# Happy-ZZX/PL-VIWO

Hardware: AMD Instinct MI355X
Metric: frames/sec (track+EKF update), 752x480 mono, 250 pts+80 lines; ATE vs CPU ref (higher is better)
Workload: dtype f64

## Files before the change

include/plviwo.h:

```cpp
#ifndef PLVIWO_H
#define PLVIWO_H

#include <stddef.h>
#include <stdint.h>

#ifdef __cplusplus
extern "C" {
#endif

#if defined(__GNUC__)
#pragma GCC visibility push(default)
#endif

#define PLV_ABI_VERSION 1

enum {
  PLV_OK = 0,
  PLV_E_BADARG = -1,
  PLV_E_DEVICE = -2,
  PLV_E_NOT_PSD = -3,
  PLV_E_NOMEM = -4,
  PLV_E_CAPACITY = -5,
  PLV_E_NO_DEVICE = -6,
  PLV_E_NUMERIC = -7
// ... 224 lines not shown
  const double *line_FinG;
  const int *D;
  const double *anchor_pt;
  const uint8_t *has_pt;
  const double *res_R;
  const double *res_p;
  const double *res_Q;
  const int *res_clone;
} plv_line_tracks;

int plv_triangulate_lines(plv_ctx *ctx, const plv_state_view *st, const plv_line_tracks *lt, double *line_FinG,
                          uint8_t *ok);

int plv_line_segments(plv_ctx *ctx, const plv_state_view *st, const plv_line_tracks *lt, double *end_points ,
                      double *extent , int *n_views , uint8_t *ok );

int plv_line_jacobian_columns(const plv_state_view *st, const plv_line_tracks *lt, int *col_to_state, int cap, int *k_out);

int plv_build_line_jacobians(plv_ctx *ctx, const plv_state_view *st, const plv_line_tracks *lt, int k,
                             const int *col_to_state, int ld, int *rows, double *Hf, double *Hx, double *res);
int plv_build_line_jacobians_resident(plv_ctx *ctx, const plv_state_view *st, const plv_line_tracks *lt, int k,
                                      const int *col_to_state, int ld);

int plv_detect_lines(plv_ctx *ctx, int which, float *lines, int cap, int *n_out);
int plv_line_prefetch_mode(plv_ctx *ctx, int on);
int plv_line_worker_config(int spin_us, int fit_threads, int *spin_us_out, int *fit_threads_out);
int plv_line_tracker_feed_async(plv_ctx *ctx, double timestamp, const double *vps);
int plv_line_tracker_feed_wait(plv_ctx *ctx);
int plv_line_detect_launch(plv_ctx *ctx, int which);
int plv_line_detect_finish(plv_ctx *ctx, int which);
int plv_line_walk_mode(plv_ctx *ctx, int on_device);
int plv_line_walk_info(plv_ctx *ctx, int *mode, int *n_components, int *longest_component, int *n_chains, int *fell_back);
int plv_line_chains(plv_ctx *ctx, int cap_chains, int cap_pts, int *chain_ptr, int *pts_xy, int *n_chains);

int plv_assign_points_to_lines(const float *lines, int n_lines, const float *pts, const uint64_t *ids, int n_pts, int *kept,
                               int *rel_ptr, uint64_t *rel_id, double *rel_dist, int *pos_ptr, float *pos_xy, int *n_kept);
int plv_line_match(const float *lines_new, int n_new, const int *rel_ptr_new, const uint64_t *rel_id_new, const float *lines_last,
                   int n_last, const int *rel_ptr_last, const uint64_t *rel_id_last, int *match_of_new);
int plv_line_classification(const float *line, const double *vps);
int plv_vanishing_points(const double *R_ItoC, const double *K8, double *vps);

int plv_line_tracker_feed(plv_ctx *ctx, double timestamp, const double *vps);
int plv_line_tracker_feed_points(plv_ctx *ctx, double timestamp, const double *vps, int n, const float *pts, const uint64_t *ids);
int plv_line_tracker_last(plv_ctx *ctx, float *lines, uint64_t *ids, int cap, int *n);
int plv_line_db_size(plv_ctx *ctx);
int plv_line_db_ids(plv_ctx *ctx, uint64_t *ids, int cap, int *n);
int plv_line_db_export_tracks(plv_ctx *ctx, const uint64_t *ids, int n_ids, int *obs_ptr, double *obs_time, float *seg_uv,
                              float *seg_uvn, int obs_cap, int *D, int *pts_ptr, int *pt_ids, int pts_cap);
int plv_line_db_remove(plv_ctx *ctx, const uint64_t *ids, int n_ids);

int plv_db_append_measurements(plv_ctx *ctx, uint64_t id, int n, const double *t, const float *uv, const float *uvn);

typedef struct plv_update_options {
  int max_msckf;
  int max_obs;
  double chi2_mult;
  plv_tri_options tri;
  double t_prev_frame;
  double state_time;
  int window_full;
  int max_slam;
  int n_slam;
  const uint64_t *slam_ids;
  int init_min_meas;
  const plv_cpi_table *cpi;
} plv_update_options;
// ... 278 lines not shown
```

pl-viwo_amd/__init__.py:

```python
import ctypes as C
import os

import numpy as np

_HERE = os.path.dirname(os.path.abspath(__file__))
LIB_PATH = os.path.join(_HERE, "lib", "libplviwo_hip.so")

PLV_OK = 0
PLV_E_BADARG = -1
PLV_E_DEVICE = -2
PLV_E_NOT_PSD = -3
PLV_E_NOMEM = -4
PLV_E_CAPACITY = -5
PLV_E_NO_DEVICE = -6
PLV_E_NUMERIC = -7

PLV_CAM_RADTAN = 0
PLV_CAM_EQUIDISTANT = 1
ENCODINGS = {"mono8": 0, "bayer_rggb8": 1, "bayer_bggr8": 2, "bayer_gbrg8": 3, "bayer_grbg8": 4, "bgr8": 5, "rgb8": 6, "bgra8": 7,
             "rgba8": 8}
_ENC_BPP = (1, 1, 1, 1, 1, 3, 3, 4, 4)


class PlvConfig(C.Structure):
# ... 188 lines not shown
        "plv_debug_knobs": (C.c_uint, [C.c_longlong]),
        "plv_chain_count": (C.c_ulonglong, []),
        "plv_decision_trace": (C.c_int, [C.c_void_p, C.c_int]),
        "plv_last_point_decisions": (C.c_int, [C.c_void_p, C.POINTER(C.c_uint64), C.POINTER(C.c_double), C.c_int, C.POINTER(C.c_int)]),
        "plv_last_line_decisions": (C.c_int, [C.c_void_p, C.POINTER(C.c_uint64), C.POINTER(C.c_double), C.c_int, C.POINTER(C.c_int)]),
        "plv_route_counts": (None, [C.POINTER(C.c_ulonglong)]),
        "plv_speculation_counts": (None, [C.POINTER(C.c_ulonglong)]),
        "plv_memory_bytes": (None, [C.POINTER(C.c_ulonglong)]),
        "plv_memory_policy": (C.c_int, [C.c_int, C.c_int, C.c_int]),
        "plv_alloc_count": (C.c_ulonglong, []),
        "plv_phase_counters": (None, [C.POINTER(C.c_ulonglong)]),
        "plv_camera_update_lines": (C.c_int, [vp, C.POINTER(PlvStateView), C.POINTER(PlvUpdateOptions), dp,
                                              C.POINTER(PlvUpdateResult), u64p, u8p, dp, C.c_int]),
        "plv_slam_update": (C.c_int, [vp, C.c_int, C.c_int, C.c_int, dp, dp, ip, C.c_double, u8p, dp]),
        "plv_slam_initialize": (C.c_int, [vp, C.c_int, C.c_int, C.c_int, dp, dp, dp, ip, C.c_double, u8p, dp, dp]),
        "plv_cov_marginalize": (C.c_int, [vp, C.c_int, C.c_int]),
        "plv_landmark_from_xyz": (C.c_int, [C.c_int, dp, dp]),
        "plv_landmark_xyz": (C.c_int, [C.c_int, dp, dp]),
        "plv_camera_update_slam": (C.c_int, [vp, C.POINTER(PlvStateView), C.POINTER(PlvUpdateOptions), C.c_int, vp, C.c_int, vp,
                                             C.POINTER(PlvTracks), C.POINTER(PlvSlamResult), u64p, u8p, dp]),
        "plv_camera_init_slam": (C.c_int, [vp, C.POINTER(PlvStateView), C.POINTER(PlvUpdateOptions), C.c_int, vp, ip, C.c_int, vp,
                                           C.POINTER(PlvTracks), C.POINTER(PlvSlamResult), u64p, u8p, dp]),
        "plv_detect_lines": (C.c_int, [vp, C.c_int, fp, C.c_int, ip]),
        "plv_line_detect_launch": (C.c_int, [vp, C.c_int]),
        "plv_line_detect_finish": (C.c_int, [vp, C.c_int]),
        "plv_counters": (None, [C.POINTER(C.c_ulonglong)]),
        "plv_jpl_left_update": (None, [C.c_int, dp, dp, dp]),
        "plv_state_boxplus": (C.c_int, [C.c_int, C.POINTER(PlvStateVar), dp, C.c_int]),
        "plv_camera_try_update": (C.c_int, [vp, C.POINTER(PlvStateView), C.POINTER(PlvTryUpdate)]),
        "plv_camera_frame": (C.c_int, [vp, C.POINTER(PlvStateView), C.POINTER(PlvCameraFrameIo)]),
        "plv_line_walk_mode": (C.c_int, [vp, C.c_int]),
        "plv_line_walk_info": (C.c_int, [vp, ip, ip, ip, ip, ip]),
        "plv_line_chains": (C.c_int, [vp, C.c_int, C.c_int, ip, ip, ip]),
        "plv_line_prefetch_mode": (C.c_int, [vp, C.c_int]),
        "plv_line_tracker_feed_async": (C.c_int, [vp, C.c_double, dp]),
        "plv_line_tracker_feed_wait": (C.c_int, [vp]),
        "plv_assign_points_to_lines": (C.c_int, [fp, C.c_int, fp, u64p, C.c_int, ip, ip, u64p, dp, ip, fp, ip]),
        "plv_line_match": (C.c_int, [fp, C.c_int, ip, u64p, fp, C.c_int, ip, u64p, ip]),
        "plv_line_classification": (C.c_int, [fp, dp]),
        "plv_vanishing_points": (C.c_int, [dp, dp, dp]),
        "plv_line_tracker_feed": (C.c_int, [vp, C.c_double, dp]),
        "plv_line_tracker_feed_points": (C.c_int, [vp, C.c_double, dp, C.c_int, fp, u64p]),
        "plv_line_tracker_last": (C.c_int, [vp, fp, u64p, C.c_int, ip]),
        "plv_line_tracker_last_points": (C.c_int, [vp, ip, u64p, C.c_int, C.c_int, ip]),
        "plv_draw_primitives": (C.c_int, [vp, u8p, C.c_int, C.c_int, C.c_int, C.POINTER(PlvDrawPrim), C.c_int, u8p, C.c_int, u8p, C.c_int]),
        "plv_track_image_options_default": (None, [C.POINTER(PlvTrackImageOptions)]),
        "plv_track_image": (C.c_int, [vp, C.POINTER(PlvTrackImageOptions), u8p, C.c_int]),
        "plv_track_image_primitives": (C.c_int, [vp, C.POINTER(PlvTrackImageOptions), C.POINTER(PlvDrawPrim), C.c_int, ip]),
        "plv_line_db_size": (C.c_int, [vp]),
        "plv_line_db_ids": (C.c_int, [vp, u64p, C.c_int, ip]),
        "plv_line_db_export_tracks": (C.c_int, [vp, u64p, C.c_int, ip, dp, fp, fp, C.c_int, ip, ip, ip, C.c_int]),
        "plv_line_db_remove": (C.c_int, [vp, u64p, C.c_int]),
        "plv_triangulate_lines": (C.c_int, [vp, C.POINTER(PlvStateView), C.POINTER(PlvLineTracks), dp, u8p]),
        "plv_line_segments": (C.c_int, [vp, C.POINTER(PlvStateView), C.POINTER(PlvLineTracks), dp, dp, ip, u8p]),
        "plv_line_map_mode": (C.c_int, [vp, C.c_int]),
        "plv_camera_used_lines": (C.c_int, [vp, C.POINTER(PlvStateView), C.c_int, ip, u64p, u8p, dp, dp, u8p]),
        "plv_line_jacobian_columns": (C.c_int, [C.POINTER(PlvStateView), C.POINTER(PlvLineTracks), ip, C.c_int, ip]),
        "plv_build_line_jacobians": (C.c_int, [vp, C.POINTER(PlvStateView), C.POINTER(PlvLineTracks), C.c_int, ip, C.c_int, ip,
                                               dp, dp, dp]),
        "plv_build_line_jacobians_resident": (C.c_int, [vp, C.POINTER(PlvStateView), C.POINTER(PlvLineTracks), C.c_int, ip,
                                                        C.c_int]),
    }
    for name, (res, args) in sig.items():
        fn = getattr(lib, name)
        fn.restype = res
        fn.argtypes = args
# ... 1331 lines not shown
            self._chk(self.lib.plv_last_point_decisions(self.h, ids.ctypes.data_as(C.POINTER(C.c_uint64)), vals.ctypes.data_as(C.POINTER(C.c_double)),
                                                        n.value, C.byref(n)))
        return ids, vals

    def last_line_decisions(self):
        n = C.c_int(0)
        self._chk(self.lib.plv_last_line_decisions(self.h, None, None, 0, C.byref(n)))
        ids, vals = np.zeros(n.value, dtype=np.uint64), np.zeros((n.value, 3))
        if n.value:
            self._chk(self.lib.plv_last_line_decisions(self.h, ids.ctypes.data_as(C.POINTER(C.c_uint64)), vals.ctypes.data_as(C.POINTER(C.c_double)),
                                                       n.value, C.byref(n)))
        return ids, vals

    def line_prefetch_mode(self, on):
        self._chk(self.lib.plv_line_prefetch_mode(self.h, 1 if on else 0))

    def line_walk_mode(self, on_device):
        self._chk(self.lib.plv_line_walk_mode(self.h, int(on_device)))

    def line_walk_info(self):
        v = [C.c_int() for _ in range(5)]
        self._chk(self.lib.plv_line_walk_info(self.h, *[C.byref(x) for x in v]))
        return dict(zip(("mode", "n_components", "longest_component", "n_chains", "fell_back"), (x.value for x in v)))

    def line_chains(self):
        n = C.c_int()
        self._chk(self.lib.plv_line_chains(self.h, 0, 0, None, None, C.byref(n)))
        ptr = np.zeros(n.value + 1, dtype=np.int32)
        self._chk(self.lib.plv_line_chains(self.h, n.value, 0, _ip(ptr), None, C.byref(n)))
        pts = np.zeros((max(int(ptr[-1]), 1), 2), dtype=np.int32)
        self._chk(self.lib.plv_line_chains(self.h, n.value, int(ptr[-1]), _ip(ptr), _ip(pts), C.byref(n)))
        return [pts[ptr[c]:ptr[c + 1]].copy() for c in range(n.value)]

    def assign_points_to_lines(self, lines, pts, ids):
        lines = np.ascontiguousarray(lines, dtype=np.float32).reshape(-1, 4)
        pts = np.ascontiguousarray(pts, dtype=np.float32).reshape(-1, 2)
        ids = np.ascontiguousarray(ids, dtype=np.uint64)
        nl, npt = len(lines), len(pts)
        kept = np.zeros(max(nl, 1), dtype=np.int32)
        rel_ptr, pos_ptr = np.zeros(nl + 1, dtype=np.int32), np.zeros(nl + 1, dtype=np.int32)
        rel_id, rel_d = np.zeros(nl * npt + 1, dtype=np.uint64), np.zeros(nl * npt + 1)
        pos = np.zeros((nl * npt + 1, 2), dtype=np.float32)
        nk = C.c_int()
        self._chk(self.lib.plv_assign_points_to_lines(_fp(lines), nl, _fp(pts), _u64p(ids), npt, _ip(kept), _ip(rel_ptr), _u64p(rel_id),
                                                      _dp(rel_d), _ip(pos_ptr), _fp(pos), C.byref(nk)))
        nk = nk.value
        return dict(kept=kept[:nk].copy(), rel_ptr=rel_ptr[:nk + 1].copy(), rel_id=rel_id[:rel_ptr[nk]].copy(),
                    rel_dist=rel_d[:rel_ptr[nk]].copy(), pos_ptr=pos_ptr[:nk + 1].copy(), pos=pos[:pos_ptr[nk]].copy())

    def line_match(self, lines_new, rel_ptr_new, rel_id_new, lines_last, rel_ptr_last, rel_id_last):
        ln = np.ascontiguousarray(lines_new, dtype=np.float32).reshape(-1, 4)
        ll = np.ascontiguousarray(lines_last, dtype=np.float32).reshape(-1, 4)
        rpn, rpl = _i32(rel_ptr_new), _i32(rel_ptr_last)
        rin = np.ascontiguousarray(rel_id_new, dtype=np.uint64)
        ril = np.ascontiguousarray(rel_id_last, dtype=np.uint64)
        out = np.zeros(max(1, len(ln)), dtype=np.int32)
        self._chk(self.lib.plv_line_match(_fp(ln), len(ln), _ip(rpn), _u64p(rin), _fp(ll), len(ll), _ip(rpl), _u64p(ril), _ip(out)))
        return out[:len(ln)].copy()

    def line_classification(self, line, vps):
        line = np.ascontiguousarray(line, dtype=np.float32)
        vps = np.ascontiguousarray(vps, dtype=np.float64)
        return self.lib.plv_line_classification(_fp(line), _dp(vps))

    def vanishing_points(self, R_ItoC, K8):
        R = np.ascontiguousarray(R_ItoC, dtype=np.float64)
# ... 246 lines not shown
```

pl-viwo_amd/csrc/line_api.hip:

```cpp
#include <algorithm>
#include <chrono>
#include <cmath>
#include <cstring>
#include <atomic>
#include <condition_variable>
#include <functional>
#include <memory>
#include <map>
#include <mutex>
#include <thread>
#include <unordered_map>
#include <vector>

#include "line_host.hpp"
#include "cam_models.hpp"
#include "line_kernels.hpp"
#include "update_state.hpp"
#include "plv_internal.hpp"
#include "camera_tracks.hpp"
#include "update_tail.hpp"

using namespace plv;
using namespace plv::linehost;

// ... 35 lines not shown
  std::vector<int> ptr, D, valid_n, cols, pt_ptr, pt_ids;
  std::vector<double> anchor, ot;
  std::vector<float> uv, uvn;
  std::vector<uint8_t> has, flags;
  CpiPoses cpi;
  std::vector<double> lg_two_step;
  std::vector<uint8_t> ok_two_step;
  double us_pool = 0;
  plv_line_tracks view() const {
    plv_line_tracks all{};
    all.n_lines = Lp, all.obs_ptr = ptr.data(), all.obs_time = ot.data(), all.seg_uv = uv.data(), all.seg_uvn = uvn.data();
    all.D = D.data(), all.anchor_pt = anchor.data(), all.has_pt = has.data();
    if (cpi.on && !cpi.R.empty()) all.res_R = cpi.R.data(), all.res_p = cpi.p.data();
    return all;
  }
};

struct LineTracker {
  LinePool pool_prep;
  LinesJob ujob;
  std::vector<float> lines_last;
  std::vector<uint64_t> ids_last;
  std::vector<int> rel_ptr_last{0};
  std::vector<uint64_t> rel_id_last;
  uint64_t currid = 1;
  bool walk_on_device = false;
  int walk_mode = 0;
  struct WalkInfo {
    int mode = 0, n_components = 0, longest_component = 0, n_chains = 0, fell_back = 0;
  } winfo;
  bool chains_valid = false;
  std::vector<FldChain> last_chains;
  int last_pts_extent = 0;
  DevBuf comps, recs, recs_sorted;
  bool prefetch = false;
  std::unordered_map<uint64_t, LineTrack> db;
  DevBuf half, map, work, pts, chains, counts, segs, seg_count, uv_in, uv_out;
  DevBuf lab, lab_cnt, lab_roots;
  hipStream_t ccl_stream = nullptr;
  hipEvent_t canny_done = nullptr, labels_ready = nullptr;
  PinBuf pin;
  hipEvent_t edges_ready = nullptr;
  std::vector<uint64_t> dec_ids;
  std::vector<double> dec_vals;
  struct LineMapRecord {
    std::vector<uint64_t> ids;
    std::vector<uint8_t> accepted;
    std::vector<double> lines, res_R, res_p;
    std::vector<int> sel, ptr;
    std::vector<double> ot;
    std::vector<float> uv, uvn;
  } map_rec;
  const uint8_t *early_raw = nullptr;
  const unsigned *early_hist = nullptr;
  int early_w = 0, early_h = 0;
  int pending_which = -1, pending_fed = -1;
  bool defer_finish = false;
  std::function<void()> deferred;
  std::atomic<int> defer_state{0};
  struct TriState {
    bool valid = false;
    plv_state_view view;
    std::vector<double> clone_time, clone_R, clone_p;
    std::vector<int> clone_id;
  } tri_state;
  std::vector<float> cached;
// ... 196 lines not shown
  TRY(T->work.reserve(npix));
  TRY(T->pts.reserve(npix * sizeof(int2)));
  TRY(T->chains.reserve(kChainCap * sizeof(FldChain)));
  TRY(T->counts.reserve(12 * sizeof(int)));
  const size_t slot_cap = npix / (size_t)fp.length_threshold + kChainCap;
  TRY(T->segs.reserve(slot_cap * sizeof(float4)));
  TRY(T->seg_count.reserve(kChainCap * sizeof(int)));
  FldBuffers b{T->half.as<uint8_t>(), T->map.as<uint8_t>(), T->work.as<uint8_t>(), T->pts.as<int2>(), T->chains.as<FldChain>(),
               kChainCap,             T->counts.as<int>(),  T->segs.as<float4>(), T->seg_count.as<int>()};
  const size_t bytes = 16 + kChainCap * (sizeof(FldChain) + sizeof(int));
  const size_t lab_off = bytes + ((2 * npix + 63) & ~(size_t)63) + npix * sizeof(int2);
  const size_t nblk = (npix + 255) / 256, sorted_off = (lab_off + npix + 63) & ~(size_t)63, bins_off = sorted_off + nblk * 256;
  const size_t pin_end = bins_off + nblk * (size_t)(plv::line_label_parts() + 1) * sizeof(unsigned short);
  const size_t info_off = (std::max(bytes + slot_cap * sizeof(float4), pin_end + 64) + 63) & ~(size_t)63;
  TRY(T->pin.reserve(info_off + 64));
  char *hp = T->pin.as<char>();
  const bool maps_to_host = !T->walk_on_device && fp.canny_low == fp.canny_high;
  if (maps_to_host) {
    b.map = (uint8_t *)(hp + bytes);
    b.half = b.map + npix;
  }
  const bool with_labels = launch_only && maps_to_host;
  if (with_labels) {
    TRY(T->lab.reserve(npix * sizeof(int)));
    TRY(T->lab_cnt.reserve(npix * sizeof(int)));
    TRY(T->lab_roots.reserve(plv::line_label_roots_bytes()));
    b.lab_work = T->lab.as<int>();
    b.lab_cnt = T->lab_cnt.as<int>();
    b.lab_roots = T->lab_roots.as<int>();
    b.lab_out = (uint8_t *)(hp + lab_off);
    b.blk_sorted = (uint8_t *)(hp + sorted_off);
    b.blk_bins = (unsigned short *)(hp + bins_off);
  }
  const bool comp_walk = T->walk_mode == 2 && fp.canny_low == fp.canny_high && plv::line_walk_lds_bytes(w, h) <= plv::kLineWalkLdsMax;
  if (comp_walk) {
    (void)join_job(T);
    const size_t rec_cap = npix / (size_t)(std::max(1, fp.length_threshold) + 1) + 1;
    TRY(T->lab.reserve(npix * sizeof(int)));
    TRY(T->lab_cnt.reserve(npix * sizeof(int)));
    TRY(T->lab_roots.reserve(plv::line_label_roots_bytes()));
    TRY(T->comps.reserve((size_t)plv::line_walk_components_cap() * sizeof(FldComp)));
    TRY(T->recs.reserve(rec_cap * sizeof(FldRec)));
    TRY(T->recs_sorted.reserve(rec_cap * sizeof(FldRec)));
    b.lab_work = T->lab.as<int>();
    b.lab_cnt = T->lab_cnt.as<int>();
    b.lab_roots = T->lab_roots.as<int>();
    b.comps = T->comps.as<FldComp>();
    b.recs = T->recs.as<FldRec>();
    b.recs_sorted = T->recs_sorted.as<FldRec>();
    b.walk_info = T->counts.as<int>() + 4;
  }
  if (!prelaunched) TRY(launch_line_edges(ctx, d_img, W, H, fp, b, ctx->stream, early ? T->early_hist : nullptr));
  if (with_labels && !T->ccl_stream) {
    PLV_HIP_CHECK(hipStreamCreateWithFlags(&T->ccl_stream, hipStreamNonBlocking));
    PLV_HIP_CHECK(hipEventCreateWithFlags(&T->canny_done, hipEventDisableTiming));
    PLV_HIP_CHECK(hipEventCreateWithFlags(&T->labels_ready, hipEventDisableTiming));
  }
  if (with_labels) PLV_HIP_CHECK(hipEventRecord(T->canny_done, ctx->stream));
  if (launch_only && !T->edges_ready) PLV_HIP_CHECK(hipEventCreateWithFlags(&T->edges_ready, hipEventDisableTiming));
  if (launch_only && maps_to_host) PLV_HIP_CHECK(hipEventRecord(T->edges_ready, ctx->stream));
  if (early && ctx->after_edges) TRY(ctx->after_edges(ctx->after_edges_arg));
  if (with_labels) {
    PLV_HIP_CHECK(hipStreamWaitEvent(T->ccl_stream, T->canny_done, 0));
    TRY(launch_line_labels(ctx, w, h, b, T->ccl_stream, fp.length_threshold));
    PLV_HIP_CHECK(hipEventRecord(T->labels_ready, T->ccl_stream));
  }
  const float thr2 = ctx->cfg.line_min_length_px * ctx->cfg.line_min_length_px;
  auto emit = [&](const float4 &sg) {
    const float x1 = sg.x * 2, y1 = sg.y * 2, x2 = sg.z * 2, y2 = sg.w * 2;
    const float l2 = (x2 - x1) * (x2 - x1) + (y2 - y1) * (y2 - y1);
    if (!(l2 > thr2)) return;
    lines.insert(lines.end(), {x1, y1, x2, y2});
  };
  lines.clear();
  if (!T->walk_on_device) {
    const bool timing = plv::knob(plv::PLV_KNOB_LINE_TIMING);
    if (prelaunched) {
      const bool had = join_job(T);
      if (had && T->job.rc == PLV_OK) {
        lines.swap(T->job.lines);
        return PLV_OK;
      }
      if (had && T->job.rc != PLV_OK) return T->job.rc;
    } else {
      (void)join_job(T);
    }
    plv::linehost::quiesce_helpers(T->host.fit);
    Job &J = T->job;
    J.device = ctx->device, J.w = w, J.h = h, J.length_threshold = fp.length_threshold, J.distance_threshold = fp.distance_threshold;
    J.thr2 = thr2;
    uint8_t *hmap = (uint8_t *)(hp + bytes);
    J.hmap = hmap, J.hhalf = hmap + npix;
    J.hpts = (int2 *)(hp + bytes + ((2 * npix + 63) & ~(size_t)63));
    J.hc = (FldChain *)(hp + 16);
    J.hlab = with_labels ? b.lab_out : nullptr;
    J.parts = with_labels ? plv::line_label_parts() : 0;
    J.hsorted = with_labels ? b.blk_sorted : nullptr, J.hbins = with_labels ? b.blk_bins : nullptr;
    if (!maps_to_host) {
      PLV_HIP_CHECK(plv::memcpy_async(hmap, T->map.p, npix, hipMemcpyDeviceToHost, ctx->stream));
      PLV_HIP_CHECK(plv::memcpy_async(hmap + npix, T->half.p, npix, hipMemcpyDeviceToHost, ctx->stream));
    }
    if (launch_only) {
      if (!maps_to_host) PLV_HIP_CHECK(hipEventRecord(T->edges_ready, ctx->stream));
      T->pending_which = which;
      T->pending_fed = plv_front_fed_count(ctx) + (early ? 1 : 0);
      if (!T->worker.joinable()) T->worker = std::thread(line_worker, T);
      {
        std::lock_guard<std::mutex> lk(T->jm);
        T->job_state = 1;
        T->job_posted = std::chrono::steady_clock::now();
      }
      T->jcv.notify_all();
      prewake_helpers(&T->host);
      return PLV_OK;
    }
    PLV_HIP_CHECK(plv::stream_sync(ctx->stream));
    TRY(host_extract(&T->host, J, timing));
    lines.swap(J.lines);
    ctx->prof.collect();
    return PLV_OK;
  }
  int *hinfo = (int *)(hp + info_off);
  if (comp_walk) {
    TRY(launch_line_walk_components(ctx, w, h, fp, b));
    TRY(launch_line_walk(ctx, w, h, fp, b, b.walk_info + 2));
    TRY(launch_line_fit(ctx, w, h, fp, b, b.walk_info + 2));
    PLV_HIP_CHECK(plv::memcpy_async(hinfo, b.walk_info, 8 * sizeof(int), hipMemcpyDeviceToHost, ctx->stream));
  } else {
    TRY(launch_line_walk(ctx, w, h, fp, b));
// ... 87 lines not shown
  if (n_components) *n_components = T->winfo.n_components;
  if (longest_component) *longest_component = T->winfo.longest_component;
  if (n_chains) *n_chains = T->winfo.n_chains;
  if (fell_back) *fell_back = T->winfo.fell_back;
  return PLV_OK;
}

int plv_line_chains(plv_ctx *ctx, int cap_chains, int cap_pts, int *chain_ptr, int *pts_xy, int *n_chains) {
  if (!ctx || cap_chains < 0 || cap_pts < 0) return PLV_E_BADARG;
  (void)hipSetDevice(ctx->device);
  LineTracker *T = ltr(ctx);
  std::lock_guard<std::mutex> lk(T->mtx);
  if (!T->chains_valid) {
    set_last_error("plv_line_chains: the last detection did not run on the device (plv_line_walk_mode 1 or 2)");
    return PLV_E_BADARG;
  }
  const int n = (int)T->last_chains.size();
  size_t total = 0;
  for (const FldChain &c : T->last_chains) total += (size_t)c.len;
  if (n_chains) *n_chains = n;
  if (!chain_ptr) return PLV_OK;
  if (n > cap_chains || (pts_xy && total > (size_t)cap_pts)) return PLV_E_CAPACITY;
  chain_ptr[0] = 0;
  for (int c = 0; c < n; ++c) chain_ptr[c + 1] = chain_ptr[c] + T->last_chains[c].len;
  if (!pts_xy || total == 0) return PLV_OK;
  std::vector<int2> hp((size_t)T->last_pts_extent);
  PLV_HIP_CHECK(plv::memcpy_async(hp.data(), T->pts.p, hp.size() * sizeof(int2), hipMemcpyDeviceToHost, ctx->stream));
  PLV_HIP_CHECK(plv::stream_sync(ctx->stream));
  for (int c = 0; c < n; ++c) {
    const FldChain &ch = T->last_chains[c];
    if (ch.start < 0 || (size_t)ch.start + (size_t)ch.len > hp.size()) return PLV_E_DEVICE;
    for (int q = 0; q < ch.len; ++q) pts_xy[2 * ((size_t)chain_ptr[c] + q)] = hp[(size_t)ch.start + q].x, pts_xy[2 * ((size_t)chain_ptr[c] + q) + 1] = hp[(size_t)ch.start + q].y;
  }
  return PLV_OK;
}

int plv_line_worker_config(int spin_us, int fit_threads_n, int *spin_us_out, int *fit_threads_out) {
  if (spin_us >= 0) spin_budget_us().store(spin_us);
  if (fit_threads_n >= 0) fit_threads().store(std::min(fit_threads_n, (int)plv::linehost::Fit::kThreads));
  if (spin_us_out) *spin_us_out = spin_budget_us().load();
  if (fit_threads_out) *fit_threads_out = fit_threads().load();
  return PLV_OK;
}

int plv_line_prefetch_mode(plv_ctx *ctx, int on) {
  if (!ctx) return PLV_E_BADARG;
  LineTracker *T = ltr(ctx);
  std::lock_guard<std::mutex> lk(T->mtx);
  T->prefetch = on != 0;
  return PLV_OK;
}
}
namespace plv {
int plv_line_prefetch_enabled(plv_ctx *ctx) {
  {
    std::lock_guard<std::mutex> lk(g_mtx);
    if (g_lt.find(ctx) == g_lt.end()) return 0;
  }
  LineTracker *T = ltr(ctx);
  std::lock_guard<std::mutex> lk(T->mtx);
  return T->prefetch && !T->walk_on_device ? 1 : 0;
}
}
extern "C" {

int plv_detect_lines(plv_ctx *ctx, int which, float *lines, int cap, int *n_out) {
// ... 891 lines not shown
```

pl-viwo_amd/csrc/line_kernels.hip:

```cpp
#include "line_kernels.hpp"

#include "fld_fit_core.hpp"
#include "equalize_lut.hpp"

namespace plv {

__global__ void __launch_bounds__(256) half_kernel(const uint8_t *__restrict__ src, int w, int h, uint8_t *__restrict__ dst) {
  const int w2 = w >> 1, h2 = h >> 1;
  const int x = blockIdx.x * 64 + (threadIdx.x & 63), y = blockIdx.y * 4 + (threadIdx.x >> 6);
  if (x >= w2 || y >= h2) return;
  const uint8_t *p = src + (size_t)(2 * y) * w + 2 * x;
  dst[(size_t)y * w2 + x] = (uint8_t)((p[0] + p[1] + p[w] + p[w + 1] + 2) >> 2);
}

#define CN_T 16
__device__ __forceinline__ int ccl_find(const int *L, int i) {
  for (;;) {
    const int p = __atomic_load_n(L + i, __ATOMIC_RELAXED);
    if (p == i) return i;
    i = p;
  }
}
__device__ __forceinline__ void ccl_union(int *L, int a, int b) {
  for (;;) {
// ... 85 lines not shown
    const int me = ty * CN_T + tx;
    const bool edge = inside && out == 2;
    lab[me] = edge ? me : -1;
    lcnt[me] = 0;
    __syncthreads();
    if (edge) {
      if (tx > 0 && lab[me - 1] >= 0) ccl_union(lab, me, me - 1);
      if (ty > 0) {
        if (tx > 0 && lab[me - CN_T - 1] >= 0) ccl_union(lab, me, me - CN_T - 1);
        if (lab[me - CN_T] >= 0) ccl_union(lab, me, me - CN_T);
        if (tx + 1 < CN_T && lab[me - CN_T + 1] >= 0) ccl_union(lab, me, me - CN_T + 1);
      }
    }
    __syncthreads();
    int r = -1;
    if (edge) {
      r = ccl_find(lab, me);
      atomicAdd(&lcnt[r], 1);
    }
    __syncthreads();
    if (inside) {
      lab_init[(size_t)y * w + x] = edge ? (y0 + r / CN_T) * w + x0 + (r & (CN_T - 1)) : -1;
      if (cnt_init) cnt_init[(size_t)y * w + x] = lcnt[me];
    }
  }
}

#define CCL_BIG 8
#define CCL_HASHED 16
#define CCL_ROOT_CAP 4096
#define CCL_PARTS (CCL_BIG + CCL_HASHED)
__global__ void __launch_bounds__(256) ccl_boundary_kernel(int *__restrict__ L, int w, int h, int *__restrict__ n_roots) {
  const int i = blockIdx.x * 256 + threadIdx.x;
  if (i == 0) *n_roots = 0;
  if (i >= w * h || L[i] < 0) return;
  const int y = i / w, x = i - y * w;
  const int lx = x & (CN_T - 1), ly = y & (CN_T - 1);
  if (lx == 0 && x > 0 && L[i - 1] >= 0) ccl_union(L, i, i - 1);
  if (y > 0) {
    if ((lx == 0 || ly == 0) && x > 0 && L[i - w - 1] >= 0) ccl_union(L, i, i - w - 1);
    if (ly == 0 && L[i - w] >= 0) ccl_union(L, i, i - w);
    if ((ly == 0 || lx == CN_T - 1) && x + 1 < w && L[i - w + 1] >= 0) ccl_union(L, i, i - w + 1);
  }
}
__global__ void __launch_bounds__(256) ccl_roots_kernel(int *__restrict__ L, int n, int *__restrict__ cnt, int *__restrict__ roots, int *__restrict__ n_roots) {
  const int i = blockIdx.x * 256 + threadIdx.x;
  if (i >= n || L[i] < 0) return;
  const int r = ccl_find(L, i);
  if (r != i) {
    __atomic_store_n(L + i, r, __ATOMIC_RELAXED);
    const int c = cnt[i];
    if (c > 0) {
      atomicAdd(cnt + r, c);
      cnt[i] = 0;
    }
  }
  if (r == i) {
    const int at = atomicAdd(n_roots, 1);
    if (at < CCL_ROOT_CAP) roots[at] = i;
  }
}
__global__ void __launch_bounds__(1024) ccl_assign_kernel(int *__restrict__ cnt, const int *__restrict__ roots, const int *__restrict__ n_roots, int min_px) {
  __shared__ int lsz[512], lrt[512];
  __shared__ int n_large;
  const int n = min(*n_roots, CCL_ROOT_CAP);
  const bool listed = *n_roots <= CCL_ROOT_CAP;
  if (threadIdx.x == 0) n_large = 0;
  __syncthreads();
  for (int j = threadIdx.x; j < n; j += blockDim.x) {
    const int root = roots[j], c = cnt[root];
    bool large = false;
    if (listed && c >= 64) {
      const int at = atomicAdd(&n_large, 1);
      if (at < 512) lsz[at] = c, lrt[at] = root, large = true;
    }
    if (!large) cnt[root] = c < min_px ? -255 : -(1 + CCL_BIG + (int)(((unsigned)root * 2654435761u >> 8) % (unsigned)CCL_HASHED));
  }
  __syncthreads();
  const int m = min(n_large, 512);
  for (int j = threadIdx.x; j < m; j += blockDim.x) {
    const int mine = lsz[j], root = lrt[j];
    int rank = 0;
    for (int q = 0; q < m && rank < CCL_BIG; ++q) rank += (lsz[q] > mine) || (lsz[q] == mine && lrt[q] < root);
    cnt[root] = -(rank < CCL_BIG ? 1 + rank : 1 + CCL_BIG + (int)(((unsigned)root * 2654435761u >> 8) % (unsigned)CCL_HASHED));
  }
}
__global__ void __launch_bounds__(256) ccl_flatten_kernel(const int *__restrict__ L, int n, const int *__restrict__ cnt, uint8_t *__restrict__ lab_out, int min_px,
                                                          uint8_t *__restrict__ blk_sorted, unsigned short *__restrict__ blk_bins) {
  __shared__ unsigned short wcnt[4][CCL_PARTS], start[CCL_PARTS + 1];
  const int i = blockIdx.x * 256 + threadIdx.x;
  uint8_t v = 0;
  if (i < n) {
    const int r = L[i];
    if (r >= 0) {
      const int c = cnt[r];
      v = (uint8_t)(c < 0 ? -c : (c < min_px ? 255 : 1 + CCL_BIG + (int)(((unsigned)r * 2654435761u >> 8) % (unsigned)CCL_HASHED)));
    }
    lab_out[i] = v;
  }
  if (!blk_sorted) return;
  const int part = (v >= 1 && v <= CCL_PARTS) ? v - 1 : -1, wave = threadIdx.x >> 6, lane = threadIdx.x & 63;
  int before = 0;
  for (int p = 0; p < CCL_PARTS; ++p) {
    const unsigned long long m = __ballot(part == p);
    if (part == p) before = __popcll(m & ((1ull << lane) - 1ull));
    if (lane == 0) wcnt[wave][p] = (unsigned short)__popcll(m);
  }
  __syncthreads();
  if (wave == 0) {
    int tot = lane < CCL_PARTS ? wcnt[0][lane] + wcnt[1][lane] + wcnt[2][lane] + wcnt[3][lane] : 0, inc = tot;
#pragma unroll
    for (int off = 1; off < 32; off <<= 1) {
      const int o = __shfl_up(inc, off, 64);
      if (lane >= off) inc += o;
    }
    if (lane < CCL_PARTS) start[lane + 1] = (unsigned short)inc;
    if (lane == 0) start[0] = 0;
  }
  __syncthreads();
  if (threadIdx.x <= CCL_PARTS) blk_bins[(size_t)blockIdx.x * (CCL_PARTS + 1) + threadIdx.x] = start[threadIdx.x];
  if (part >= 0) {
    int at = start[part] + before;
    for (int w = 0; w < wave; ++w) at += wcnt[w][part];
    blk_sorted[(size_t)blockIdx.x * 256 + at] = (uint8_t)threadIdx.x;
  }
}

__global__ void __launch_bounds__(1024) canny_hyst_kernel(uint8_t *__restrict__ map, int w, int h) {
  __shared__ int changed;
  do {
    __syncthreads();
    if (threadIdx.x == 0) changed = 0;
// ... 443 lines not shown
}

static inline int cdiv(int a, int b) { return (a + b - 1) / b; }

int launch_line_edges(plv_ctx *ctx, const uint8_t *d_img, int W, int H, const FldParams &fp, FldBuffers &b, hipStream_t st, const unsigned *d_hist) {
  if (!st) st = ctx->stream;
  const int w = W / 2, h = H / 2;
  int low = fp.canny_low, high = fp.canny_high;
  if (low > high) std::swap(low, high);
  {
    ProfScope ps(ctx->prof, "half_canny_kernel", st);
    hipLaunchKernelGGL(canny_kernel<true>, dim3(cdiv(w, CN_T), cdiv(h, CN_T)), dim3(CN_T * CN_T), 0, st, d_img, W, w, h, low,
                       high, b.map, b.half, d_hist, W * H, b.lab_work, b.lab_cnt);
  }
  if (low != high) {
    ProfScope ps(ctx->prof, "canny_hyst_kernel", st);
    hipLaunchKernelGGL(canny_hyst_kernel, dim3(1), dim3(1024), 0, st, b.map, w, h);
  }
  PLV_HIP_CHECK(hipGetLastError());
  return PLV_OK;
}

int launch_line_labels(plv_ctx *ctx, int w, int h, FldBuffers &b, hipStream_t st, int length_threshold) {
  const int n = w * h;
  const int min_px = length_threshold + 1;
  {
    ProfScope ps(ctx->prof, "ccl_boundary_kernel", st);
    hipLaunchKernelGGL(ccl_boundary_kernel, dim3(cdiv(n, 256)), dim3(256), 0, st, b.lab_work, w, h, b.lab_roots + CCL_ROOT_CAP);
  }
  {
    ProfScope ps(ctx->prof, "ccl_roots_kernel", st);
    hipLaunchKernelGGL(ccl_roots_kernel, dim3(cdiv(n, 256)), dim3(256), 0, st, b.lab_work, n, b.lab_cnt, b.lab_roots, b.lab_roots + CCL_ROOT_CAP);
  }
  {
    ProfScope ps(ctx->prof, "ccl_assign_kernel", st);
    hipLaunchKernelGGL(ccl_assign_kernel, dim3(1), dim3(1024), 0, st, b.lab_cnt, b.lab_roots, b.lab_roots + CCL_ROOT_CAP, min_px);
  }
  {
    ProfScope ps(ctx->prof, "ccl_flatten_kernel", st);
    hipLaunchKernelGGL(ccl_flatten_kernel, dim3(cdiv(n, 256)), dim3(256), 0, st, b.lab_work, n, b.lab_cnt, b.lab_out, min_px, b.blk_sorted, b.blk_bins);
  }
  PLV_HIP_CHECK(hipGetLastError());
  return PLV_OK;
}
int line_label_parts() { return CCL_PARTS; }
size_t line_label_roots_bytes() { return (CCL_ROOT_CAP + 4) * sizeof(int); }

int launch_line_walk(plv_ctx *ctx, int w, int h, const FldParams &fp, FldBuffers &b, const int *gate) {
  ProfScope ps(ctx->prof, "fld_walk_kernel", ctx->stream);
  const size_t need = (size_t)w * h;
  if (need <= 150 * 1024) {
    PLV_HIP_CHECK(ensure_dyn_smem((const void *)fld_walk_kernel<true>, (int)need));
    hipLaunchKernelGGL(fld_walk_kernel<true>, dim3(1), dim3(64), need, ctx->stream, b.map, w, h, fp.length_threshold, b.work, b.pts,
                       b.chains, b.chain_cap, b.counts, gate);
  } else {
    hipLaunchKernelGGL(fld_walk_kernel<false>, dim3(1), dim3(64), 0, ctx->stream, b.map, w, h, fp.length_threshold, b.work, b.pts,
                       b.chains, b.chain_cap, b.counts, gate);
  }
  PLV_HIP_CHECK(hipGetLastError());
  return PLV_OK;
}

int launch_line_fit(plv_ctx *ctx, int w, int h, const FldParams &fp, FldBuffers &b, const int *gate) {
  ProfScope ps(ctx->prof, "fld_fit_kernel", ctx->stream);
  hipLaunchKernelGGL(fld_fit_kernel, dim3(cdiv(b.chain_cap, 64)), dim3(64), 0, ctx->stream, b.half, w, h, fp.length_threshold,
                     fp.distance_threshold, b.pts, b.chains, b.counts, b.segs, b.seg_count, gate);
  PLV_HIP_CHECK(hipGetLastError());
  return PLV_OK;
}

size_t line_walk_lds_bytes(int w, int h) { return (size_t)h * (size_t)((w + 63) / 64) * sizeof(unsigned long long); }
int line_walk_components_cap() { return CCL_ROOT_CAP; }
int launch_line_walk_components(plv_ctx *ctx, int w, int h, const FldParams &fp, FldBuffers &b) {
  hipStream_t st = ctx->stream;
  const int n = w * h, min_px = fp.length_threshold + 1;
  const size_t lds = line_walk_lds_bytes(w, h);
  if (lds > kLineWalkLdsMax || !b.lab_work || !b.comps) return PLV_E_BADARG;
  {
    ProfScope ps(ctx->prof, "ccl_boundary_kernel", st);
// ... 36 lines not shown
```

pl-viwo_amd/csrc/plv_ctx.hpp:

```cpp
#pragma once
#include <hip/hip_runtime.h>
#include <sys/resource.h>

#include "gate_stage.hpp"
#include <cstdint>
#include <cstdio>
#include <execinfo.h>
#include <cstring>
#include <algorithm>
#include <atomic>
#include <chrono>
#include <cstdlib>
#include <mutex>
#include <string>
#include <unordered_map>
#include <vector>

#include "../../include/plviwo.h"

namespace plv {

void set_last_error(const char *fmt, ...);

#define PLV_HIP_CHECK(expr)                                                              \
// ... 15 lines not shown
  std::atomic<unsigned long long> speculated{0};
  std::atomic<unsigned long long> route[8] = {};
};
inline Counters &counters() {
  static Counters c;
  return c;
}
inline int spec_grid(int max_sel) { return 2 * (max_sel > 0 ? max_sel : 1); }
inline hipError_t stream_sync(hipStream_t s) {
  ++counters().syncs;
  return hipStreamSynchronize(s);
}
inline hipError_t event_sync(hipEvent_t e) {
  ++counters().syncs;
  return hipEventSynchronize(e);
}
inline hipError_t memcpy_async(void *dst, const void *src, size_t bytes, hipMemcpyKind kind, hipStream_t s) {
  ++counters().copies;
  counters().copy_bytes += bytes;
  return hipMemcpyAsync(dst, src, bytes, kind, s);
}

enum : unsigned { PLV_KNOB_PRIOR_LATE = 2u, PLV_KNOB_GATE_SEPARATE = 1024u, PLV_KNOB_NO_CHAIN = 2048u, PLV_KNOB_CHAIN_ALWAYS = 4096u,
                  PLV_KNOB_FORCE_FACTOR_FORM = 8192u,
                  PLV_KNOB_HOST_TIMING = 1u << 14,
                  PLV_KNOB_LINE_TIMING = 1u << 15,
                  PLV_KNOB_UPDATE_TIMING = 1u << 16,
                  PLV_KNOB_KERNEL_STAMPS = 1u << 17,
                  PLV_KNOB_CHAIN_EVENTS = 1u << 18,
                  PLV_KNOB_ALLOC_DEBUG = 1u << 19,
                  PLV_KNOB_HOST_FAULTS = 1u << 20,
                  PLV_KNOB_NO_SPECULATION = 1u << 24,
                  PLV_KNOB_HELPER_NAPS = 1u << 28,
                  PLV_KNOB_TSQR_TREE = 1u << 29 };
inline std::atomic<unsigned> &knobs() {
  static std::atomic<unsigned> k{getenv("PLV_DEBUG_KNOBS") ? (unsigned)strtoul(getenv("PLV_DEBUG_KNOBS"), nullptr, 0) : 0u};
  return k;
}
inline bool knob(unsigned bit) { return (knobs().load(std::memory_order_relaxed) & bit) != 0; }
inline bool alloc_debug() { return knob(PLV_KNOB_ALLOC_DEBUG); }

struct HostPhases {
  struct Rec {
    const char *label;
    double us = 0;
    long n = 0;
    float last[64] = {};
    void put(double v) {
      last[n & 63] = (float)v;
      us += v;
      ++n;
    }
    double median() const {
      float tmp[64];
      const int m = (int)(n < 64 ? n : 64);
      for (int i = 0; i < m; ++i) tmp[i] = last[i];
      std::sort(tmp, tmp + m);
      return m ? tmp[m / 2] : 0.0;
    }
  };
  bool on = knob(PLV_KNOB_HOST_TIMING);
  std::mutex mtx;
  std::vector<Rec> recs;
  void add(const char *label, double us) {
    std::lock_guard<std::mutex> lk(mtx);
    for (auto &r : recs)
      if (r.label == label) {
// ... 367 lines not shown
```

Measured before the change: 2203.

## Parallelize CCL root assignment across workgroups and rank large components in flatten

Replaces the single-1024-thread-workgroup component assignment kernel with a multi-workgroup kernel. Large components are appended to a list via an atomic counter, and their final rank is computed inside the flatten kernel by comparing against an LDS copy of the large-component keys. This removes a serial single-WG step in connected-component labelling, at the cost of extra per-pixel rank work and LDS use in flatten. Adds a plv_line_parts API to read back the labels, and a debug knob that restores the old single-WG path.

After: 2168. 0.984x the previous value.

```diff
diff --git a/include/plviwo.h b/include/plviwo.h
--- a/include/plviwo.h
+++ b/include/plviwo.h
@@ -280,6 +280,7 @@
 int plv_line_walk_mode(plv_ctx *ctx, int on_device);
 int plv_line_walk_info(plv_ctx *ctx, int *mode, int *n_components, int *longest_component, int *n_chains, int *fell_back);
 int plv_line_chains(plv_ctx *ctx, int cap_chains, int cap_pts, int *chain_ptr, int *pts_xy, int *n_chains);
+int plv_line_parts(plv_ctx *ctx, uint8_t *parts, int cap, int *n_out);
 
 int plv_assign_points_to_lines(const float *lines, int n_lines, const float *pts, const uint64_t *ids, int n_pts, int *kept,
                                int *rel_ptr, uint64_t *rel_id, double *rel_dist, int *pos_ptr, float *pos_xy, int *n_kept);
diff --git a/pl-viwo_amd/__init__.py b/pl-viwo_amd/__init__.py
--- a/pl-viwo_amd/__init__.py
+++ b/pl-viwo_amd/__init__.py
@@ -244,6 +244,7 @@
         "plv_line_walk_mode": (C.c_int, [vp, C.c_int]),
         "plv_line_walk_info": (C.c_int, [vp, ip, ip, ip, ip, ip]),
         "plv_line_chains": (C.c_int, [vp, C.c_int, C.c_int, ip, ip, ip]),
+        "plv_line_parts": (C.c_int, [vp, vp, C.c_int, ip]),
         "plv_line_prefetch_mode": (C.c_int, [vp, C.c_int]),
         "plv_line_tracker_feed_async": (C.c_int, [vp, C.c_double, dp]),
         "plv_line_tracker_feed_wait": (C.c_int, [vp]),
@@ -1641,6 +1642,13 @@
         self._chk(self.lib.plv_line_chains(self.h, n.value, int(ptr[-1]), _ip(ptr), _ip(pts), C.byref(n)))
         return [pts[ptr[c]:ptr[c + 1]].copy() for c in range(n.value)]
 
+    def line_parts(self):
+        n = C.c_int()
+        self._chk(self.lib.plv_line_parts(self.h, None, 0, C.byref(n)))
+        out = np.zeros(n.value, dtype=np.uint8)
+        self._chk(self.lib.plv_line_parts(self.h, out.ctypes.data_as(C.c_void_p), n.value, C.byref(n)))
+        return out
+
     def assign_points_to_lines(self, lines, pts, ids):
         lines = np.ascontiguousarray(lines, dtype=np.float32).reshape(-1, 4)
         pts = np.ascontiguousarray(pts, dtype=np.float32).reshape(-1, 2)
diff --git a/pl-viwo_amd/csrc/line_api.hip b/pl-viwo_amd/csrc/line_api.hip
--- a/pl-viwo_amd/csrc/line_api.hip
+++ b/pl-viwo_amd/csrc/line_api.hip
@@ -91,6 +91,7 @@
   bool chains_valid = false;
   std::vector<FldChain> last_chains;
   int last_pts_extent = 0;
+  size_t parts_off = 0, parts_n = 0;
   DevBuf comps, recs, recs_sorted;
   bool prefetch = false;
   std::unordered_map<uint64_t, LineTrack> db;
@@ -353,6 +354,7 @@
     b.blk_sorted = (uint8_t *)(hp + sorted_off);
     b.blk_bins = (unsigned short *)(hp + bins_off);
   }
+  if (!prelaunched) T->parts_off = lab_off, T->parts_n = with_labels ? npix : 0;
   const bool comp_walk = T->walk_mode == 2 && fp.canny_low == fp.canny_high && plv::line_walk_lds_bytes(w, h) <= plv::kLineWalkLdsMax;
   if (comp_walk) {
     (void)join_job(T);
@@ -414,8 +416,7 @@
     J.hmap = hmap, J.hhalf = hmap + npix;
     J.hpts = (int2 *)(hp + bytes + ((2 * npix + 63) & ~(size_t)63));
     J.hc = (FldChain *)(hp + 16);
-    J.hlab = with_labels ? b.lab_out : nullptr;
-    J.parts = with_labels ? plv::line_label_parts() : 0;
+    J.hlab = with_labels ? b.lab_out : nullptr;    J.parts = with_labels ? plv::line_label_parts() : 0;
     J.hsorted = with_labels ? b.blk_sorted : nullptr, J.hbins = with_labels ? b.blk_bins : nullptr;
     if (!maps_to_host) {
       PLV_HIP_CHECK(plv::memcpy_async(hmap, T->map.p, npix, hipMemcpyDeviceToHost, ctx->stream));
@@ -569,6 +570,23 @@
     if (ch.start < 0 || (size_t)ch.start + (size_t)ch.len > hp.size()) return PLV_E_DEVICE;
     for (int q = 0; q < ch.len; ++q) pts_xy[2 * ((size_t)chain_ptr[c] + q)] = hp[(size_t)ch.start + q].x, pts_xy[2 * ((size_t)chain_ptr[c] + q) + 1] = hp[(size_t)ch.start + q].y;
   }
+  return PLV_OK;
+}
+
+int plv_line_parts(plv_ctx *ctx, uint8_t *parts, int cap, int *n_out) {
+  if (!ctx || cap < 0) return PLV_E_BADARG;
+  (void)hipSetDevice(ctx->device);
+  LineTracker *T = ltr(ctx);
+  std::lock_guard<std::mutex> lk(T->mtx);
+  if (T->parts_n == 0 || !T->ccl_stream) {
+    set_last_error("plv_line_parts: the last detection was not labelled (plv_line_detect_launch, equal Canny thresholds, walk mode 0)");
+    return PLV_E_BADARG;
+  }
+  if (n_out) *n_out = (int)T->parts_n;
+  if (!parts) return PLV_OK;
+  if (T->parts_n > (size_t)cap) return PLV_E_CAPACITY;
+  PLV_HIP_CHECK(plv::stream_sync(T->ccl_stream));
+  std::memcpy(parts, T->pin.as<char>() + T->parts_off, T->parts_n);
   return PLV_OK;
 }
 
diff --git a/pl-viwo_amd/csrc/line_kernels.hip b/pl-viwo_amd/csrc/line_kernels.hip
--- a/pl-viwo_amd/csrc/line_kernels.hip
+++ b/pl-viwo_amd/csrc/line_kernels.hip
@@ -141,7 +141,7 @@
 #define CCL_PARTS (CCL_BIG + CCL_HASHED)
 __global__ void __launch_bounds__(256) ccl_boundary_kernel(int *__restrict__ L, int w, int h, int *__restrict__ n_roots) {
   const int i = blockIdx.x * 256 + threadIdx.x;
-  if (i == 0) *n_roots = 0;
+  if (i == 0) n_roots[0] = 0, n_roots[1] = 0;
   if (i >= w * h || L[i] < 0) return;
   const int y = i / w, x = i - y * w;
   const int lx = x & (CN_T - 1), ly = y & (CN_T - 1);
@@ -169,7 +169,27 @@
     if (at < CCL_ROOT_CAP) roots[at] = i;
   }
 }
-__global__ void __launch_bounds__(1024) ccl_assign_kernel(int *__restrict__ cnt, const int *__restrict__ roots, const int *__restrict__ n_roots, int min_px) {
+#define CCL_LARGE_PX 64
+#define CCL_LARGE_CAP 512
+#define CCL_LARGE_BASE 256
+__device__ __forceinline__ int ccl_hashed_part(int root) { return 1 + CCL_BIG + (int)(((unsigned)root * 2654435761u >> 8) % (unsigned)CCL_HASHED); }
+__global__ void __launch_bounds__(256) ccl_assign_kernel(int *__restrict__ cnt, const int *__restrict__ roots, int *__restrict__ n_roots, int min_px,
+                                                         int2 *__restrict__ large) {
+  const int nr = n_roots[0], j = blockIdx.x * 256 + threadIdx.x;
+  if (j >= min(nr, CCL_ROOT_CAP)) return;
+  const bool listed = nr <= CCL_ROOT_CAP;
+  const int root = roots[j], c = cnt[root];
+  if (listed && c >= CCL_LARGE_PX) {
+    const int at = atomicAdd(n_roots + 1, 1);
+    if (at < CCL_LARGE_CAP) {
+      large[at] = make_int2(c, root);
+      cnt[root] = -(CCL_LARGE_BASE + at);
+      return;
+    }
+  }
+  cnt[root] = c < min_px ? -255 : -ccl_hashed_part(root);
+}
+__global__ void __launch_bounds__(1024) ccl_assign_one_kernel(int *__restrict__ cnt, const int *__restrict__ roots, const int *__restrict__ n_roots, int min_px) {
   __shared__ int lsz[512], lrt[512];
   __shared__ int n_large;
   const int n = min(*n_roots, CCL_ROOT_CAP);
@@ -195,18 +215,35 @@
   }
 }
 __global__ void __launch_bounds__(256) ccl_flatten_kernel(const int *__restrict__ L, int n, const int *__restrict__ cnt, uint8_t *__restrict__ lab_out, int min_px,
-                                                          uint8_t *__restrict__ blk_sorted, unsigned short *__restrict__ blk_bins) {
+                                                          uint8_t *__restrict__ blk_sorted, unsigned short *__restrict__ blk_bins,
+                                                          const int2 *__restrict__ large, const int *__restrict__ n_large) {
   __shared__ unsigned short wcnt[4][CCL_PARTS], start[CCL_PARTS + 1];
+  __shared__ unsigned long long lkey[CCL_LARGE_CAP];
   const int i = blockIdx.x * 256 + threadIdx.x;
+  const int r = i < n ? L[i] : -1;
+  const int c = r >= 0 ? cnt[r] : 0;
+  const int m = min(*n_large, CCL_LARGE_CAP), m4 = (m + 3) & ~3;
+  if (m > 0) {
+    for (int j = threadIdx.x; j < m4; j += 256) {
+      const int2 e = j < m ? large[j] : make_int2(0, 0x7fffffff);
+      lkey[j] = ((unsigned long long)(unsigned)e.x << 32) | (unsigned)(0x7fffffff - e.y);
+    }
+    __syncthreads();
+  }
   uint8_t v = 0;
-  if (i < n) {
-    const int r = L[i];
-    if (r >= 0) {
-      const int c = cnt[r];
-      v = (uint8_t)(c < 0 ? -c : (c < min_px ? 255 : 1 + CCL_BIG + (int)(((unsigned)r * 2654435761u >> 8) % (unsigned)CCL_HASHED)));
-    }
-    lab_out[i] = v;
-  }
+  if (r >= 0) {
+    const int at = -c - CCL_LARGE_BASE;
+    if (at >= 0 && at < m) {
+      const unsigned long long mine = lkey[at];
+      int rank = 0;
+      for (int q = 0; q < m4; q += 4)
+        rank += (int)(lkey[q] > mine) + (int)(lkey[q + 1] > mine) + (int)(lkey[q + 2] > mine) + (int)(lkey[q + 3] > mine);
+      v = (uint8_t)(rank < CCL_BIG ? 1 + rank : ccl_hashed_part(r));
+    } else {
+      v = (uint8_t)(c < 0 ? -c : (c < min_px ? 255 : ccl_hashed_part(r)));
+    }
+  }
+  if (i < n) lab_out[i] = v;
   if (!blk_sorted) return;
   const int part = (v >= 1 && v <= CCL_PARTS) ? v - 1 : -1, wave = threadIdx.x >> 6, lane = threadIdx.x & 63;
   int before = 0;
@@ -716,19 +753,25 @@
     ProfScope ps(ctx->prof, "ccl_roots_kernel", st);
     hipLaunchKernelGGL(ccl_roots_kernel, dim3(cdiv(n, 256)), dim3(256), 0, st, b.lab_work, n, b.lab_cnt, b.lab_roots, b.lab_roots + CCL_ROOT_CAP);
   }
+  int *n_roots = b.lab_roots + CCL_ROOT_CAP;
+  int2 *large = (int2 *)(b.lab_roots + CCL_ROOT_CAP + 4);
   {
     ProfScope ps(ctx->prof, "ccl_assign_kernel", st);
-    hipLaunchKernelGGL(ccl_assign_kernel, dim3(1), dim3(1024), 0, st, b.lab_cnt, b.lab_roots, b.lab_roots + CCL_ROOT_CAP, min_px);
+    if (plv::knob(plv::PLV_KNOB_ASSIGN_ONE_WG))
+      hipLaunchKernelGGL(ccl_assign_one_kernel, dim3(1), dim3(1024), 0, st, b.lab_cnt, b.lab_roots, n_roots, min_px);
+    else
+      hipLaunchKernelGGL(ccl_assign_kernel, dim3(CCL_ROOT_CAP / 256), dim3(256), 0, st, b.lab_cnt, b.lab_roots, n_roots, min_px, large);
   }
   {
     ProfScope ps(ctx->prof, "ccl_flatten_kernel", st);
-    hipLaunchKernelGGL(ccl_flatten_kernel, dim3(cdiv(n, 256)), dim3(256), 0, st, b.lab_work, n, b.lab_cnt, b.lab_out, min_px, b.blk_sorted, b.blk_bins);
+    hipLaunchKernelGGL(ccl_flatten_kernel, dim3(cdiv(n, 256)), dim3(256), 0, st, b.lab_work, n, b.lab_cnt, b.lab_out, min_px, b.blk_sorted, b.blk_bins, large,
+                       n_roots + 1);
   }
   PLV_HIP_CHECK(hipGetLastError());
   return PLV_OK;
 }
 int line_label_parts() { return CCL_PARTS; }
-size_t line_label_roots_bytes() { return (CCL_ROOT_CAP + 4) * sizeof(int); }
+size_t line_label_roots_bytes() { return (CCL_ROOT_CAP + 4) * sizeof(int) + CCL_LARGE_CAP * sizeof(int2); }
 
 int launch_line_walk(plv_ctx *ctx, int w, int h, const FldParams &fp, FldBuffers &b, const int *gate) {
   ProfScope ps(ctx->prof, "fld_walk_kernel", ctx->stream);
diff --git a/pl-viwo_amd/csrc/plv_ctx.hpp b/pl-viwo_amd/csrc/plv_ctx.hpp
--- a/pl-viwo_amd/csrc/plv_ctx.hpp
+++ b/pl-viwo_amd/csrc/plv_ctx.hpp
@@ -71,7 +71,8 @@
                   PLV_KNOB_HOST_FAULTS = 1u << 20,
                   PLV_KNOB_NO_SPECULATION = 1u << 24,
                   PLV_KNOB_HELPER_NAPS = 1u << 28,
-                  PLV_KNOB_TSQR_TREE = 1u << 29 };
+                  PLV_KNOB_TSQR_TREE = 1u << 29,
+                  PLV_KNOB_ASSIGN_ONE_WG = 1u << 30 };
 inline std::atomic<unsigned> &knobs() {
   static std::atomic<unsigned> k{getenv("PLV_DEBUG_KNOBS") ? (unsigned)strtoul(getenv("PLV_DEBUG_KNOBS"), nullptr, 0) : 0u};
   return k;
```
